# Sanoojan/REFace

Hardware: AMD Instinct MI355X
Metric: 512x512 50-step DDIM images/sec (higher is better)
Workload: dtype bf16; 1 GPU; BASELINE configs[1]: 512x512, 50 DDIM steps, CFG scale 3.5, batch 8 per GPU, bf16 UNet + fp32 VAE decode (bf16x3 MFMA operands), seeded random-init REFace weights; id=c1:512x512:S50:B8:bf16, batch_per_gpu=8, global_batch=8, ddim_steps=50, latent=64, parallelism=dp1 (pairs sharded, no collective in the step loop)

## Files before the change

### include/reface_hip.h

```cpp
#ifndef REFACE_HIP_H
#define REFACE_HIP_H

#include <stdint.h>

#ifdef __cplusplus
extern "C" {
#endif

enum { RF_F32 = 0, RF_BF16 = 1, RF_FP8_E4M3 = 2 ,
       RF_BF16X3 = 3 ,
       RF_F16 = 4  };

enum { RF_ACT_NONE = 0, RF_ACT_GEGLU = 1, RF_ACT_SILU = 2, RF_ACT_QUICK_GELU = 3, RF_ACT_GELU = 4,
       RF_ACT_RELU = 5, RF_ACT_SIGMOID = 6, RF_ACT_PRELU = 7, RF_ACT_ADD_RELU = 8 };

const char* rf_last_error(void);
int rf_version(void);

typedef struct rf_conv_gemm_desc {
    int32_t dtype;
    int32_t out_dtype;
    int32_t M, N, K;
    const void* src0;
    const void* src1;
// ... 73 lines not shown
    void* x1; int32_t ldx1;
} rf_ffn_desc;
int rf_ffn_block(const rf_ffn_desc* d, void* stream);

typedef struct rf_attn_in_desc {
    const void* x; int32_t ldx;
    const void* wpi; int64_t w_sample_stride;
    const float* rowvec; int32_t ldv, rows_per_sample;
    void* tok; int32_t ldt;
    const void* wqkv; const float* bqkv;
    void* qkv; int32_t ldq;
    int32_t M, C;
    float ln_eps;
    int32_t dtype;
} rf_attn_in_desc;
int rf_attn_in(const rf_attn_in_desc* d, void* stream);

int rf_quantize_fp8_rows(const float* w, int N, int K, int ldq, void* q, float* scale, void* stream);

int rf_groupnorm_stats(int dtype, const void* x, int B, int HW, int C, int ldx, int nchunks, double* partial, void* stream);
int rf_groupnorm_finalize(const double* partial_in, int B, int nchunks, double* partial_out, void* stream);
int rf_groupnorm_apply(int dtype, const void* x, int B, int HW, int C, int ldx, int nchunks, const double* partial,
                       const float* gamma, const float* beta, float eps, int silu, int out_dtype, void* out, int ldo, void* stream);
int rf_groupnorm_fold_linear(const float* W, int N, int C, int B, int HW, int nchunks, const double* partial, const float* gamma, const float* beta,
                             const float* bias, float eps, int out_dtype, void* w_out, float* rowvec_out, void* stream);

int rf_gn_silu_conv3x3_small(int dtype, const void* x, int B, int H, int W, int C, int ldx, int nchunks, const double* partial, const float* gamma,
                             const float* beta, float eps, int silu, const void* w, const float* bias, int No, int out_dtype, void* out, int ldo,
                             float* workspace, long long workspace_bytes, void* stream);

typedef struct rf_stem_desc {
    const void* x; int32_t ldx;
    int32_t B, H, W, C;
    const void* w; const float* bias;
    void* out; int32_t ldo;
    long long dup_off;
    double* gn_part0;
    int32_t gn_cpg0, gn_coff0, gn_slot0, gn_nchunks0;
    double* gn_part1;
    int32_t gn_cpg1, gn_coff1, gn_slot1, gn_nchunks1;
    double* gn_part2;
    int32_t gn_cpg2, gn_coff2, gn_slot2, gn_nchunks2;
    int32_t dtype;
} rf_stem_desc;
int rf_conv3x3_stem(const rf_stem_desc* d, void* stream);

// ... 151 lines not shown
```

### reface_amd/_lib.py

```python
import ctypes as C
import os

HERE = os.path.dirname(os.path.abspath(__file__))
LIB_PATH = os.environ.get("REFACE_HIP_LIB") or os.path.join(HERE, "lib", "libreface_hip.so")

RF_F32, RF_BF16, RF_FP8_E4M3, RF_BF16X3, RF_F16 = 0, 1, 2, 3, 4
ACT_NONE, ACT_GEGLU, ACT_SILU, ACT_QUICK_GELU, ACT_GELU, ACT_RELU, ACT_SIGMOID, ACT_PRELU, ACT_ADD_RELU = 0, 1, 2, 3, 4, 5, 6, 7, 8


class ConvGemmDesc(C.Structure):
    _fields_ = [
        ("dtype", C.c_int32), ("out_dtype", C.c_int32),
        ("M", C.c_int32), ("N", C.c_int32), ("K", C.c_int32),
        ("src0", C.c_void_p), ("src1", C.c_void_p),
        ("C0", C.c_int32), ("C1", C.c_int32), ("ld0", C.c_int32), ("ld1", C.c_int32),
        ("Hin", C.c_int32), ("Win", C.c_int32), ("Hout", C.c_int32), ("Wout", C.c_int32),
        ("KH", C.c_int32), ("KW", C.c_int32), ("stride", C.c_int32), ("pad_t", C.c_int32), ("pad_l", C.c_int32),
        ("ups", C.c_int32),
        ("W", C.c_void_p), ("ldw", C.c_int32), ("bias", C.c_void_p), ("rowvec", C.c_void_p),
        ("rows_per_sample", C.c_int32), ("ldv", C.c_int32),
        ("residual", C.c_void_p), ("ldr", C.c_int32), ("act", C.c_int32),
        ("out", C.c_void_p), ("ldo", C.c_int32), ("alpha", C.c_float),
        ("batch", C.c_int32),
        ("sA", C.c_int64), ("sW", C.c_int64), ("sO", C.c_int64), ("sR", C.c_int64),
# ... 58 lines not shown
        ("gn_part0", C.c_void_p), ("gn_cpg0", C.c_int32), ("gn_coff0", C.c_int32), ("gn_slot0", C.c_int32), ("gn_nchunks0", C.c_int32),
        ("gn_part1", C.c_void_p), ("gn_cpg1", C.c_int32), ("gn_coff1", C.c_int32), ("gn_slot1", C.c_int32), ("gn_nchunks1", C.c_int32),
        ("gn_part2", C.c_void_p), ("gn_cpg2", C.c_int32), ("gn_coff2", C.c_int32), ("gn_slot2", C.c_int32), ("gn_nchunks2", C.c_int32),
        ("dtype", C.c_int32),
    ]


_SIGS = {
    "rf_last_error": (C.c_char_p, []),
    "rf_version": (C.c_int, []),
    "rf_conv_gemm": (C.c_int, [C.POINTER(ConvGemmDesc), C.c_void_p]),
    "rf_conv_gemm_plan": (C.c_int, [C.POINTER(ConvGemmDesc), C.POINTER(C.c_int32), C.POINTER(C.c_int32), C.POINTER(C.c_int32)]),
    "rf_conv_gemm_plan2": (C.c_int, [C.POINTER(ConvGemmDesc), C.POINTER(C.c_int32)]),
    "rf_conv_gemm_plan3": (C.c_int, [C.POINTER(ConvGemmDesc), C.POINTER(C.c_int32)]),
    "rf_ffn_geglu": (C.c_int, [C.c_void_p, C.c_int, C.c_void_p, C.c_void_p, C.c_void_p, C.c_void_p, C.c_void_p, C.c_int, C.c_void_p, C.c_int,
                               C.c_int, C.c_int, C.c_float, C.c_void_p]),
    "rf_ffn_block": (C.c_int, [C.POINTER(FfnDesc), C.c_void_p]),
    "rf_attn_in": (C.c_int, [C.POINTER(AttnInDesc), C.c_void_p]),
    "rf_quantize_fp8_rows": (C.c_int, [C.c_void_p, C.c_int, C.c_int, C.c_int, C.c_void_p, C.c_void_p, C.c_void_p]),
    "rf_groupnorm_stats": (C.c_int, [C.c_int, C.c_void_p, C.c_int, C.c_int, C.c_int, C.c_int, C.c_int, C.c_void_p, C.c_void_p]),
    "rf_groupnorm_finalize": (C.c_int, [C.c_void_p, C.c_int, C.c_int, C.c_void_p, C.c_void_p]),
    "rf_groupnorm_apply": (C.c_int, [C.c_int, C.c_void_p, C.c_int, C.c_int, C.c_int, C.c_int, C.c_int, C.c_void_p, C.c_void_p,
                                     C.c_void_p, C.c_float, C.c_int, C.c_int, C.c_void_p, C.c_int, C.c_void_p]),
    "rf_groupnorm_fold_linear": (C.c_int, [C.c_void_p, C.c_int, C.c_int, C.c_int, C.c_int, C.c_int, C.c_void_p, C.c_void_p, C.c_void_p, C.c_void_p,
                                           C.c_float, C.c_int, C.c_void_p, C.c_void_p, C.c_void_p]),
    "rf_gn_silu_conv3x3_small": (C.c_int, [C.c_int, C.c_void_p, C.c_int, C.c_int, C.c_int, C.c_int, C.c_int, C.c_int, C.c_void_p, C.c_void_p, C.c_void_p, C.c_float, C.c_int,
                                           C.c_void_p, C.c_void_p, C.c_int, C.c_int, C.c_void_p, C.c_int, C.c_void_p, C.c_longlong, C.c_void_p]),
    "rf_conv3x3_stem": (C.c_int, [C.POINTER(StemDesc), C.c_void_p]),
    "rf_quantize_fp8_act": (C.c_int, [C.c_void_p, C.c_int64, C.c_int, C.c_int, C.c_void_p, C.c_int, C.c_void_p, C.c_int, C.c_void_p]),
    "rf_groupnorm_apply_fp8": (C.c_int, [C.c_void_p, C.c_int, C.c_int, C.c_int, C.c_int, C.c_int, C.c_void_p, C.c_void_p, C.c_void_p, C.c_float,
                                         C.c_int, C.c_void_p, C.c_int, C.c_void_p, C.c_int, C.c_void_p]),
    "rf_layernorm_fp8": (C.c_int, [C.c_void_p, C.c_int, C.c_int, C.c_int, C.c_void_p, C.c_void_p, C.c_float, C.c_void_p, C.c_int, C.c_void_p, C.c_int,
                                   C.c_void_p]),
    "rf_layernorm": (C.c_int, [C.c_int, C.c_void_p, C.c_int, C.c_int, C.c_int, C.c_void_p, C.c_void_p, C.c_float, C.c_int,
                               C.c_void_p, C.c_int, C.c_void_p]),
    "rf_attention": (C.c_int, [C.c_int, C.c_void_p, C.c_void_p, C.c_void_p, C.c_void_p, C.c_int, C.c_int, C.c_int, C.c_int, C.c_int,
                               C.c_int, C.c_int, C.c_int, C.c_int, C.c_int64, C.c_int64, C.c_int64, C.c_int64, C.c_float, C.c_void_p]),
    "rf_attention_plan": (C.c_int, [C.c_int, C.c_int, C.c_int, C.c_int, C.c_int, C.c_int, C.POINTER(C.c_int32)]),
    "rf_softmax_rows": (C.c_int, [C.c_void_p, C.c_int, C.c_int, C.c_int, C.c_void_p]),
    "rf_ddim_pack_input": (C.c_int, [C.c_void_p, C.c_void_p, C.c_void_p, C.c_int, C.c_int, C.c_int, C.c_int, C.c_void_p, C.c_int, C.c_void_p]),
    "rf_ddim_update": (C.c_int, [C.c_void_p, C.c_int, C.c_int, C.c_float, C.c_void_p, C.c_void_p, C.c_void_p, C.c_int, C.c_int,
                                 C.c_void_p, C.c_void_p]),
    "rf_dpm_update": (C.c_int, [C.c_void_p, C.c_int, C.c_int, C.c_float, C.c_void_p, C.c_void_p, C.c_void_p, C.c_int, C.c_int,
                                C.c_void_p, C.c_void_p]),
    "rf_nchw_to_nhwc": (C.c_int, [C.c_void_p, C.c_int, C.c_int, C.c_int, C.c_int, C.c_void_p, C.c_int, C.c_void_p]),
    "rf_nhwc_to_nchw": (C.c_int, [C.c_int, C.c_void_p, C.c_int, C.c_int, C.c_int, C.c_int, C.c_void_p, C.c_void_p]),
# ... 114 lines not shown
```

### reface_amd/csrc/norm.hip

```cpp
#include <stdarg.h>

#include "common.h"

namespace rf {

static thread_local char g_err[512] = "";
void set_error(const char* fmt, ...) {
    va_list ap;
    va_start(ap, fmt);
    vsnprintf(g_err, sizeof(g_err), fmt, ap);
    va_end(ap);
}

constexpr int GN_SLOTS = 4;
constexpr int GN_THREADS = 256;

template <typename T> struct gn_acc { typedef float type; };
template <> struct gn_acc<float> { typedef double type; };

template <typename T, int NS>
__global__ __launch_bounds__(GN_THREADS) void gn_stats_kernel(const T* __restrict__ x, int HW, int C, int ldx, int nchunks,
                                                              double* __restrict__ partial) {
    typedef typename gn_acc<T>::type acc_t;
    constexpr int VEC = elem<T>::VEC;
    const int nvec = C / VEC;
    const int TV = nvec < GN_THREADS ? nvec : GN_THREADS;
    const int PL = GN_THREADS / TV;
    const int tv = threadIdx.x % TV, pl = threadIdx.x / TV;
    const int b = blockIdx.y, chunk = blockIdx.x;
    const int ppc = (HW + nchunks - 1) / nchunks;
    const int p0 = chunk * ppc, p1 = min(HW, p0 + ppc);
    const int cpg = C / 32;

    constexpr bool SHIFTED = sizeof(T) == 2;
    acc_t s[NS][VEC], ss[NS][VEC];
    float k0[NS][VEC];
    int npix = 0;
#pragma unroll
    for (int q = 0; q < NS; ++q)
#pragma unroll
        for (int e = 0; e < VEC; ++e) { s[q][e] = ss[q][e] = 0; k0[q][e] = 0.f; }

    if (pl < PL) {
        int p = p0 + pl;
        if (SHIFTED && p < p1) {
            const T* row = x + ((long long)b * HW + p) * ldx;
#pragma unroll
            for (int q = 0; q < NS; ++q) {
                const int v = tv + q * TV;
                if (v < nvec) unpack16<T>(*(const u32x4_t*)(row + v * VEC), k0[q]);
            }
            npix = 1;
            p += PL;
        }
        for (; p < p1; p += PL) {
            const T* row = x + ((long long)b * HW + p) * ldx;
#pragma unroll
            for (int q = 0; q < NS; ++q) {
                const int v = tv + q * TV;
                if (v < nvec) {
                    float f[VEC];
                    unpack16<T>(*(const u32x4_t*)(row + v * VEC), f);
#pragma unroll
                    for (int e = 0; e < VEC; ++e) {
                        if constexpr (SHIFTED) {
                            const float d = f[e] - k0[q][e];
                            s[q][e] += d;
                            ss[q][e] += d * d;
                        } else {
                            s[q][e] += f[e];
                            ss[q][e] += (acc_t)f[e] * f[e];
                        }
                    }
                }
            }
            ++npix;
        }
    }
    extern __shared__ __attribute__((aligned(16))) char gn_smem[];
// ... 22 lines not shown
    __shared__ double red[GN_THREADS][2];
    {
        const int g = threadIdx.x & 31, part = threadIdx.x >> 5;
        double a = 0.0, qq = 0.0;
        const int n = PL * cpg;
        for (int e = part; e < n; e += GN_THREADS / 32) {
            const int pp = e / cpg, cc = e - pp * cpg;
            a += chs[pp * C + g * cpg + cc];
            qq += chq[pp * C + g * cpg + cc];
        }
        red[threadIdx.x][0] = a;
        red[threadIdx.x][1] = qq;
    }
    __syncthreads();
    if (threadIdx.x < 32) {
        double sa = 0.0, sq = 0.0;
        for (int k = 0; k < GN_THREADS / 32; ++k) { sa += red[threadIdx.x + 32 * k][0]; sq += red[threadIdx.x + 32 * k][1]; }
        double* o = partial + (((long long)b * nchunks + chunk) * 32 + threadIdx.x) * 2;
        o[0] = sa;
        o[1] = sq;
    }
}

template <typename T, typename TO, int NS>
__global__ __launch_bounds__(GN_THREADS) void gn_apply_kernel(const T* __restrict__ x, int HW, int C, int ldx, int nchunks,
                                                              const double* __restrict__ partial, const float* __restrict__ gamma,
                                                              const float* __restrict__ beta, float eps, int do_silu,
                                                              TO* __restrict__ out, int ldo, int achunks, int split,
                                                              fp8_t* __restrict__ sc_out = nullptr, int lds_sc = 0) {
    constexpr int VEC = elem<T>::VEC;
    const int nvec = C / VEC;
    const int TV = nvec < GN_THREADS ? nvec : GN_THREADS;
    const int PL = GN_THREADS / TV;
    const int tv = threadIdx.x % TV, pl = threadIdx.x / TV;
    const int b = blockIdx.y;
    const int cpg = C / 32;

    __shared__ float mean_s[32], rstd_s[32];
    __shared__ double red[GN_THREADS][2];
    const int ppc = (HW + achunks - 1) / achunks;
    const int p0 = blockIdx.x * ppc, p1 = min(HW, p0 + ppc);
    float gm[NS][VEC], bt[NS][VEC];
    u32x4_t raw0[NS];
#pragma unroll
    for (int q = 0; q < NS; ++q) {
        const int v = tv + q * TV;
#pragma unroll
        for (int e = 0; e < VEC; ++e) { gm[q][e] = 0.f; bt[q][e] = 0.f; }
        raw0[q] = u32x4_t{0u, 0u, 0u, 0u};
        if (v < nvec) {
#pragma unroll
            for (int e = 0; e < VEC; e += 4) {
                const f32x4_t g4 = *(const f32x4_t*)(gamma + v * VEC + e), b4 = *(const f32x4_t*)(beta + v * VEC + e);
                gm[q][e] = g4[0]; gm[q][e + 1] = g4[1]; gm[q][e + 2] = g4[2]; gm[q][e + 3] = g4[3];
                bt[q][e] = b4[0]; bt[q][e + 1] = b4[1]; bt[q][e + 2] = b4[2]; bt[q][e + 3] = b4[3];
            }
            if (pl < PL && p0 + pl < p1) raw0[q] = *(const u32x4_t*)(x + ((long long)b * HW + p0 + pl) * ldx + v * VEC);
        }
    }
    {
        const int g = threadIdx.x & 31, part = threadIdx.x >> 5;
        double a = 0.0, q = 0.0;
#pragma unroll 4
        for (int c = part; c < nchunks; c += GN_THREADS / 32) {
            const double* pp = partial + (((long long)b * nchunks + c) * 32 + g) * 2;
            a += pp[0];
            q += pp[1];
        }
        red[threadIdx.x][0] = a;
        red[threadIdx.x][1] = q;
        __syncthreads();
        if (threadIdx.x < 32) {
            double sa = 0.0, sq = 0.0;
            for (int k = 0; k < GN_THREADS / 32; ++k) { sa += red[threadIdx.x + 32 * k][0]; sq += red[threadIdx.x + 32 * k][1]; }
            const double n = (double)HW * cpg;
            const double mean = sa / n;
            double var = sq / n - mean * mean;
            if (var < 0.0) var = 0.0;
            mean_s[threadIdx.x] = (float)mean;
            rstd_s[threadIdx.x] = (float)(1.0 / sqrt(var + (double)eps));
        }
        __syncthreads();
    }
    float sc[NS][VEC], sh[NS][VEC];
#pragma unroll
    for (int q = 0; q < NS; ++q) {
        const int v = tv + q * TV;
#pragma unroll
        for (int e = 0; e < VEC; ++e) {
            sc[q][e] = sh[q][e] = 0.f;
            if (v < nvec) {
                const int c = v * VEC + e, g = c / cpg;
                const float a = rstd_s[g] * gm[q][e];
                sc[q][e] = a;
                sh[q][e] = bt[q][e] - mean_s[g] * a;
            }
        }
    }
    if (pl >= PL) return;
    u32x4_t cur[NS];
#pragma unroll
    for (int q = 0; q < NS; ++q) cur[q] = raw0[q];
    for (int p = p0 + pl; p < p1; p += PL) {
        const T* nrow = x + ((long long)b * HW + p + PL) * ldx;
        TO* orow = out + ((long long)b * HW + p) * ldo;
        u32x4_t nxt[NS];
#pragma unroll
        for (int q = 0; q < NS; ++q) {
            const int v = tv + q * TV;
            nxt[q] = u32x4_t{0u, 0u, 0u, 0u};
            if (v < nvec && p + PL < p1) nxt[q] = *(const u32x4_t*)(nrow + v * VEC);
        }
#pragma unroll
        for (int q = 0; q < NS; ++q) {
            const int v = tv + q * TV;
            if (v < nvec) {
                float f[VEC];
                unpack16<T>(cur[q], f);
#pragma unroll
                for (int e = 0; e < VEC; ++e) {
                    float y = f[e] * sc[q][e] + sh[q][e];
                    f[e] = do_silu ? silu_exact(y) : y;
                }
                if constexpr (sizeof(TO) == 1) {
                    quant_block8(f, orow + v * VEC, sc_out + ((long long)b * HW + p) * lds_sc + (v >> 2), (v & 3) == 0);
                } else if constexpr (sizeof(TO) == sizeof(T)) {
                    *(u32x4_t*)(orow + v * VEC) = pack16<TO>(f);
                } else if constexpr (sizeof(TO) == 4) {
                    *(u32x4_t*)(orow + v * VEC) = pack16<float>(f);
                    *(u32x4_t*)(orow + v * VEC + 4) = pack16<float>(f + 4);
                } else {
                    u32x2_t h, l;
                    split4_bf16(f, h, l);
                    *(u32x2_t*)(orow + v * VEC) = h;
                    if (split) *(u32x2_t*)(orow + C + v * VEC) = l;
                }
            }
        }
#pragma unroll
        for (int q = 0; q < NS; ++q) cur[q] = nxt[q];
    }
// ... 102 lines not shown
    __syncthreads();
    float s = 0.f;
    for (int c = threadIdx.x * 4; c < cols; c += 1024) {
        const f32x4_t v = *(const f32x4_t*)(r + c);
        s += expf(v[0] - m) + expf(v[1] - m) + expf(v[2] - m) + expf(v[3] - m);
    }
    s = wave_sum(s);
    if ((threadIdx.x & 63) == 0) red[threadIdx.x >> 6] = s;
    __syncthreads();
    const float inv = 1.0f / (red[0] + red[1] + red[2] + red[3]);
    for (int c = threadIdx.x * 4; c < cols; c += 1024) {
        f32x4_t v = *(const f32x4_t*)(r + c);
#pragma unroll
        for (int e = 0; e < 4; ++e) v[e] = expf(v[e] - m) * inv;
        *(f32x4_t*)(r + c) = v;
    }
}

}

using namespace rf;

extern "C" const char* rf_last_error(void) { return rf::g_err; }
extern "C" int rf_version(void) { return 111; }

static int gn_check(const char* name, int dtype, int C, int ldx, int nchunks) {
    const int vec = dtype == RF_F32 ? 4 : 8;
    RF_CHECK(dtype == RF_F32 || dtype == RF_BF16 || dtype == RF_F16, "%s: bad dtype %d", name, dtype);
    RF_CHECK(C % 32 == 0 && C % vec == 0 && ldx % vec == 0, "%s: C=%d ld=%d must be multiples of 32 and %d", name, C, ldx, vec);
    RF_CHECK(C / vec <= GN_SLOTS * GN_THREADS, "%s: C=%d too large", name, C);
    RF_CHECK(nchunks >= 1, "%s: nchunks=%d", name, nchunks);
    return 0;
}

extern "C" int rf_groupnorm_stats(int dtype, const void* x, int B, int HW, int C, int ldx, int nchunks, double* partial, void* stream) {
    if (gn_check("rf_groupnorm_stats", dtype, C, ldx, nchunks)) return 1;
    RF_CHECK(x && partial && B > 0 && HW > 0, "rf_groupnorm_stats: bad arguments");
    dim3 grid(nchunks, B);
    const int vec = dtype == RF_F32 ? 4 : 8;
    const int nvec = C / vec, TV = nvec < GN_THREADS ? nvec : GN_THREADS, PL = GN_THREADS / TV;
    const size_t smem = (size_t)2 * PL * C * sizeof(double);
    RF_CHECK(smem <= 64 * 1024, "rf_groupnorm_stats: C=%d needs %zu B of LDS", C, smem);
    const int ns = (nvec + GN_THREADS - 1) / GN_THREADS;
#define GN_STATS_(T, NS_) hipLaunchKernelGGL((gn_stats_kernel<T, NS_>), grid, dim3(GN_THREADS), smem, (hipStream_t)stream, (const T*)x, HW, C, ldx, nchunks, partial)
#define GN_STATS(T) { if (ns <= 1) GN_STATS_(T, 1); else if (ns <= 2) GN_STATS_(T, 2); else GN_STATS_(T, GN_SLOTS); }
    if (dtype == RF_F32) GN_STATS(float)
    else if (dtype == RF_F16) GN_STATS(f16_t)
// ... 42 lines not shown
    RF_CHECK(!split || (dtype == RF_F32 && ldo >= 2 * C), "rf_groupnorm_apply: split-bf16 output needs fp32 input and ldo >= 2C");
    RF_CHECK(ldo % 8 == 0, "rf_groupnorm_apply: ldo=%d must be a multiple of 8", ldo);
    int achunks = (1024 + B - 1) / B;
    const int maxc = (HW + 1) / 2;
    if (achunks > maxc) achunks = maxc;
    if (achunks < 1) achunks = 1;
    dim3 grid(achunks, B);
    hipStream_t st = (hipStream_t)stream;
    const int ns = (C / (dtype == RF_F32 ? 4 : 8) + GN_THREADS - 1) / GN_THREADS;
#define GN_APPLY_(T, TO, NS_) hipLaunchKernelGGL((gn_apply_kernel<T, TO, NS_>), grid, dim3(GN_THREADS), 0, st, (const T*)x, HW, C, ldx, nchunks, partial, gamma, beta, eps, silu, (TO*)out, ldo, achunks, split)
#define GN_APPLY(T, TO) { if (ns <= 1) GN_APPLY_(T, TO, 1); else if (ns <= 2) GN_APPLY_(T, TO, 2); else GN_APPLY_(T, TO, GN_SLOTS); }
    if (dtype == RF_F32 && out_dtype == RF_F32) GN_APPLY(float, float)
    else if (dtype == RF_F16 && out_dtype == RF_F32) GN_APPLY(f16_t, float)
    else if (dtype == RF_F16) GN_APPLY(f16_t, f16_t)
    else if (dtype == RF_F32) GN_APPLY(float, bf16_t)
    else if (out_dtype == RF_F32) GN_APPLY(bf16_t, float)
    else GN_APPLY(bf16_t, bf16_t)
#undef GN_APPLY
#undef GN_APPLY_
    RF_LAUNCH_CHECK("rf_groupnorm_apply");
    return 0;
}

constexpr int GN_FOLD_RPW = 2;
typedef float f32x2_t __attribute__((ext_vector_type(2)));
template <typename TO, int NIT>
__global__ __launch_bounds__(GN_THREADS) void gn_fold_linear_kernel(const float* __restrict__ W, int N, int C, int HW, int nchunks,
                                                                    const double* __restrict__ partial, const float* __restrict__ gamma,
                                                                    const float* __restrict__ beta, const float* __restrict__ bias, float eps,
                                                                    TO* __restrict__ wout, float* __restrict__ rvout) {
    const int b = blockIdx.y, cpg = C / 32;
    const int lane = threadIdx.x & 63, wave = threadIdx.x >> 6;
    const int n0 = (blockIdx.x * (GN_THREADS / 64) + wave) * GN_FOLD_RPW;
    f32x4_t w8[GN_FOLD_RPW][NIT][2], g8[NIT][2], b8[NIT][2];
#pragma unroll
    for (int it = 0; it < NIT; ++it) {
        const int k = 8 * lane + 512 * it;
#pragma unroll
        for (int h = 0; h < 2; ++h) {
            g8[it][h] = b8[it][h] = f32x4_t{0.f, 0.f, 0.f, 0.f};
            if (k < C) { g8[it][h] = *(const f32x4_t*)(gamma + k + 4 * h); b8[it][h] = *(const f32x4_t*)(beta + k + 4 * h); }
#pragma unroll
            for (int r = 0; r < GN_FOLD_RPW; ++r) {
                w8[r][it][h] = f32x4_t{0.f, 0.f, 0.f, 0.f};
                if (k < C && n0 + r < N) w8[r][it][h] = *(const f32x4_t*)(W + (long long)(n0 + r) * C + k + 4 * h);
            }
// ... 183 lines not shown
```

### reface_amd/ops.py

```python
import ctypes as C
import threading

import torch

from . import _lib
from ._lib import (ACT_ADD_RELU, ACT_GEGLU, ACT_GELU, ACT_NONE, ACT_PRELU, ACT_QUICK_GELU, ACT_RELU, ACT_SIGMOID, ACT_SILU, RF_BF16, RF_BF16X3, RF_F16, RF_F32,
                   RF_FP8_E4M3, AttnInDesc, ConvGemmDesc, FfnDesc, StemDesc)

LOG2E = 1.4426950408889634
LN2 = 0.6931471805599453


def code(dt):
    if dt == torch.float32:
        return RF_F32
    if dt == torch.bfloat16:
        return RF_BF16
    if dt == torch.float16:
        return RF_F16
    raise TypeError(f"unsupported dtype {dt}")


H16 = (torch.bfloat16, torch.float16)

# ... 515 lines not shown
    B, H, W_, Cc = x.shape
    n = gn_chunks(B, H * W_)
    _require_gpu(x, partial)
    assert partial.dtype == torch.float64 and partial.numel() >= B * n * 64
    return Launch(lib.rf_groupnorm_stats, (code(x.dtype), _p(x), B, H * W_, Cc, x.stride(2), n, _p(partial)), (x, partial), name + ".stats"), n


def groupnorm(x, gamma, beta, out, partial, *, eps, silu, split=False, name="groupnorm"):
    lib = _lib.load()
    B, H, W_, Cc = x.shape
    HW = H * W_
    n = gn_chunks(B, HW)
    assert partial.dtype == torch.float64 and partial.numel() >= B * n * 64
    a = Launch(lib.rf_groupnorm_stats, (code(x.dtype), _p(x), B, HW, Cc, x.stride(2), n, _p(partial)), (x, partial), name + ".stats")
    if isinstance(out, Fp8Act):
        return [a, groupnorm_apply(x, gamma, beta, out, partial, n, eps=eps, silu=silu, name=name)]
    _require_gpu(x, gamma, beta, out, partial)
    b = Launch(lib.rf_groupnorm_apply, (code(x.dtype), _p(x), B, HW, Cc, x.stride(2), n, _p(partial), _p(gamma), _p(beta),
                                        float(eps), int(bool(silu)), _gn_out_code(x, out, split), _p(out), out.stride(2)),
               (x, partial, gamma, beta, out), name + ".apply")
    return [a, b]


def gemm_plan(launch):
    pl = gemm_plan3(launch, ".plan")
    return pl["stat_rows"], pl["stat_cols"], pl["splitk"]


PLAN2_KEYS = ("stat_rows", "stat_cols", "splitk", "bm", "bn", "wave_cols", "direct", "frag", "gemm_kernels")


def gemm_plan2(launch):
    pl = gemm_plan3(launch, ".plan2")
    return {k: pl[k] for k in PLAN2_KEYS}


REDUCE_KINDS = ("none", "stripe8", "stripe32", "frag")


def gemm_plan3(launch, what=".plan3"):
    lib = _lib.load()
    info = (C.c_int32 * 24)()
    _lib.check(lib.rf_conv_gemm_plan3(C.byref(launch.keep[0]), info), launch.name + what)
    v = [int(x) for x in info]
    pl = dict(zip(PLAN2_KEYS[:8], v[:8]))
    pl["gemm_kernels"] = 2 if pl["frag"] & 2 else 1
# ... 733 lines not shown
```

### reface_amd/vae.py

```python
import os

import torch
import torch.nn as nn

from . import ops
from .gnfuse import ProducerTracker
from .modules import ParamTree, flat_state, weights_version
from .params import VAEConfig, vae_param_specs
from .unet import _Pool

F32 = torch.float32


class DiagonalGaussianDistribution(object):

    def __init__(self, parameters, deterministic=False):
        self.parameters = parameters
        self.deterministic = deterministic

    @property
    def mean(self):
        return torch.chunk(self.parameters, 2, dim=1)[0]

    @property
# ... 4 lines not shown
        B, C2, H, W = self.parameters.shape
        out = torch.empty((B, C2 // 2, H, W), dtype=F32, device=self.parameters.device)
        ops.gaussian_sample(self.parameters.contiguous(), eps, out, scale=scale)()
        return out

    def sample(self, noise=None, scale=1.0):
        if self.deterministic:
            return self._draw(None, scale)
        if noise is None:
            noise = torch.randn(self.mean.shape)
        return self._draw(noise.to(device=self.parameters.device, dtype=F32).contiguous(), scale)

    def mode(self):
        return self._draw(None, 1.0)


class _VAEEngine:
    def __init__(self, sd, cfg: VAEConfig, B, H, W, dtype, device, which):
        self.x3 = dtype == "bf16x3"
        if self.x3:
            dtype = F32
        self.cfg, self.B, self.dt, self.dev = cfg, B, dtype, device
        self.n_x3 = 0
        self.pool = _Pool(device)
        self.tracker = ProducerTracker()
        self.pool.on_put = self.tracker.forget
        self.gn_fuse = os.environ.get("REFACE_GN_FUSE", "1") == "1"
        self.gn_fused = 0
        self.sd = {k: v.detach().to(device=device, dtype=F32) for k, v in sd.items()}
        self.gn_partial = torch.empty(B * ops.GN_MAX_CHUNKS * 64, dtype=torch.float64, device=device)
        self.launches = []
        self.ws = ops.new_workspace(device)
        with ops.workspace_scope(self.ws):
            (self._build_decoder if which == "dec" else self._build_encoder)(H, W)
        self.sd = None

    def w(self, key):
        return self.sd[key].to(self.dt).contiguous()

    def f32(self, key):
        return self.sd[key].contiguous()

    def _x3_ok(self, cin, ksize=3):
        return self.x3 and ops.x3_eligible(ksize * ksize * cin, cin)

    def _split(self, x):
        B, H, W, c = x.shape
        s = self.pool.get((B, H, W, 2 * c), torch.bfloat16)
        self.launches.append(ops.split_bf16(x, s, name="split_bf16"))
        return s

    def _gn(self, x, key, silu=True, split=False):
        out = self.pool.get(tuple(x.shape[:3]) + (2 * x.shape[3],), torch.bfloat16) if split else self.pool.get(tuple(x.shape), self.dt)
# ... 13 lines not shown
        return out

    def _conv3(self, key, x, cout, *, cin_pad=None, stride=1, pad=(1, 1), ups=0, residual=None, out=None):
        B, H, W, _ = x.shape
        Ho, Wo = (2 * H, 2 * W) if ups else ((H // 2, W // 2) if stride == 2 else (H, W))
        y = out if out is not None else self.pool.get((B, Ho, Wo, cout), self.dt)
        x3 = self.x3 and x.dtype == torch.bfloat16
        wp = ops.pack_conv_weight(self.sd[key + ".weight"], F32 if x3 else self.dt, cin_pad=cin_pad)
        if x3:
            wp = ops.pack_x3(wp)
            self.n_x3 += 1
        self._conv(x, wp, y, self.f32(key + ".bias"), stride=stride, pad=pad, ups=ups, residual=residual, x3=x3, name=key)
        return y

    def _conv(self, x, wp, y, bias, residual=None, **kw):
        B, n = x.shape[0], 1
        while (x.numel() // n) * x.element_size() >= 0x7fff0000 and B % (2 * n) == 0:
            n *= 2
        step = B // n
        for i in range(n):
            sl = slice(i * step, (i + 1) * step)
            self.launches.append(self.tracker.record(y[sl], ops.conv2d(x[sl], wp, y[sl], bias, residual=None if residual is None else residual[sl], **kw)))

    def _res(self, p, x, cin, cout):
        B, H, W, _ = x.shape
        t1 = self._gn(x, f"{p}.norm1", split=self._x3_ok(cin))
        h1 = self._conv3(f"{p}.conv1", t1, cout)
        self.pool.put(t1)
        t2 = self._gn(h1, f"{p}.norm2", split=self._x3_ok(cout))
        self.pool.put(h1)
        if cin != cout:
            sc = self.pool.get((B, H, W, cout), self.dt)
            if self._x3_ok(cin, 1):
                xs = self._split(x)
                self._conv(xs, ops.pack_x3(self.sd[f"{p}.nin_shortcut.weight"].reshape(cout, cin)), sc,
                           self.f32(f"{p}.nin_shortcut.bias"), ksize=1, pad=(0, 0), x3=True, name=f"{p}.nin_shortcut")
                self.pool.put(xs)
                self.n_x3 += 1
            else:
                self._conv(x, self.w(f"{p}.nin_shortcut.weight").reshape(cout, cin), sc,
                           self.f32(f"{p}.nin_shortcut.bias"), ksize=1, pad=(0, 0), name=f"{p}.nin_shortcut")
        else:
            sc = x
        y = self._conv3(f"{p}.conv2", t2, cout, residual=sc)
        self.pool.put(t2)
        if cin != cout:
            self.pool.put(sc)
        return y

    def _attn(self, p, x, c):
        B, H, W, _ = x.shape
        N = H * W
        M = B * N
        g = self._gn(x, f"{p}.norm", silu=False)
        g2 = g.view(M, c)
        wq, wk, wv = (self.sd[f"{p}.{n}.weight"].reshape(c, c) for n in ("q", "k", "v"))
        qk = self.pool.get((M, 2 * c), self.dt)
        self.launches.append(ops.linear(g2, torch.cat([wq, wk], 0).to(self.dt).contiguous(), qk,
                                        torch.cat([self.sd[f"{p}.q.bias"], self.sd[f"{p}.k.bias"]]).contiguous(), name=f"{p}.qk"))
        vt = self.pool.get((B, c, N), self.dt)
        self.launches.append(ops.conv_gemm(wv.to(self.dt).contiguous(), g2, vt, M=c, N=N, K=c, C0=c, ld0=c, Hin=1, Win=c, Hout=1, Wout=c,
                                           ldo=N, batch=B, sA=0, sW=N * c, sO=c * N, name=f"{p}.vT"))
        scores = self.pool.get((B, N, N), F32)
        self.launches.append(ops.conv_gemm(qk, qk[:, c:], scores, M=N, N=N, K=c, C0=c, ld0=2 * c, Hin=1, Win=N, Hout=1, Wout=N,
                                           ldo=N, alpha=float(int(c) ** (-0.5)), batch=B, sA=N * 2 * c, sW=N * 2 * c, sO=N * N, ldw=2 * c,
                                           name=f"{p}.scores"))
        self.launches.append(ops.softmax_rows(scores.view(B * N, N), name=f"{p}.softmax"))
        if self.dt != F32:
            probs = self.pool.get((B, N, N), self.dt)
            self.launches.append(ops.cast(scores, probs))
# ... 20 lines not shown

    def _build_decoder(self, h, w):
        cfg, B, dev = self.cfg, self.B, self.dev
        ZP = 8
        self.z_in = torch.empty((B, cfg.embed_dim, h, w), dtype=F32, device=dev)
        z_cl = torch.zeros((B, h, w, ZP), dtype=self.dt, device=dev)
        self.launches.append(ops.nchw_to_nhwc(self.z_in, z_cl))
        zq = torch.zeros((B, h, w, ZP), dtype=self.dt, device=dev)
        wpq = torch.zeros((cfg.z_channels, ZP), dtype=F32, device=dev)
        wpq[:, :cfg.embed_dim] = self.sd["post_quant_conv.weight"].reshape(cfg.z_channels, cfg.embed_dim)
        self.pq_alpha_launch_index = len(self.launches)
        self._pq = (z_cl, wpq.to(self.dt).contiguous(), zq)
        self.launches.append(None)
        nres = len(cfg.ch_mult)
        block_in = cfg.ch * cfg.ch_mult[nres - 1]
        hcur = self._conv3("decoder.conv_in", zq, block_in, cin_pad=ZP)
        hcur = self._mid("decoder.mid", hcur, block_in)
        for lvl in reversed(range(nres)):
            block_out = cfg.ch * cfg.ch_mult[lvl]
            for b in range(cfg.num_res_blocks + 1):
                nh = self._res(f"decoder.up.{lvl}.block.{b}", hcur, block_in, block_out)
                self.pool.put(hcur)
                hcur, block_in = nh, block_out
            if lvl != 0:
                hs = self._split(hcur) if self._x3_ok(block_in) else hcur
                nh = self._conv3(f"decoder.up.{lvl}.upsample.conv", hs, block_in, ups=1)
                if hs is not hcur:
                    self.pool.put(hs)
                self.pool.put(hcur)
                hcur = nh
        g = self._gn(hcur, "decoder.norm_out", split=self._x3_ok(block_in))
        self.pool.put(hcur)
        H, W = g.shape[1], g.shape[2]
        out4 = torch.empty((B, H, W, 4), dtype=F32, device=dev)
        self._conv3("decoder.conv_out", g, cfg.out_ch, out=out4[..., :cfg.out_ch])
        self.out = torch.empty((B, cfg.out_ch, H, W), dtype=F32, device=dev)
        self.launches.append(ops.nhwc_to_nchw(out4, self.out, C_=cfg.out_ch))
        self.set_scale(1.0)

    def set_scale(self, inv_scale):
        z_cl, wpq, zq = self._pq
        B, h, w, ZP = z_cl.shape
        self.launches[self.pq_alpha_launch_index] = ops.conv_gemm(
            z_cl, wpq, zq, M=B * h * w, N=self.cfg.z_channels, K=ZP, C0=ZP, ld0=ZP, Hin=1, Win=B * h * w, Hout=1, Wout=B * h * w,
            bias=self._pq_bias(), ldo=ZP, alpha=float(inv_scale), name="post_quant_conv")

    def _pq_bias(self):
# ... 105 lines not shown
```

Before: 10.32 images/s.

## Fold VAE upsample conv into four phase 2x2 convs with phase-aware groupnorm

Replaces the nearest-upsample plus 3x3 conv in the VAE decoder with four sub-pixel phase convolutions using folded 2x2 weights. The result stays in a phase-major layout, and new groupnorm stats/apply kernels read that layout directly. The apply kernel also writes the raw fp32 or split-bf16 activations in normal layout, so the following resblock can use them for its residual or shortcut. This is meant to cut the FLOPs and memory traffic of convolving an upsampled tensor, and to remove a separate split pass. The cost is extra kernel complexity and strided gathers.

```diff
diff --git a/include/reface_hip.h b/include/reface_hip.h
--- a/include/reface_hip.h
+++ b/include/reface_hip.h
@@ -119,6 +119,10 @@
 int rf_groupnorm_finalize(const double* partial_in, int B, int nchunks, double* partial_out, void* stream);
 int rf_groupnorm_apply(int dtype, const void* x, int B, int HW, int C, int ldx, int nchunks, const double* partial,
                        const float* gamma, const float* beta, float eps, int silu, int out_dtype, void* out, int ldo, void* stream);
+int rf_groupnorm_stats_ph(const float* x, int B, int Hs, int Ws, int C, int ldx, int nchunks, double* partial, void* stream);
+int rf_groupnorm_apply_ph(const float* x, int B, int Hs, int Ws, int C, int ldx, int nchunks, const double* partial, const float* gamma,
+                          const float* beta, float eps, int silu, void* out, int ldo, float* raw_out, int ldr, void* raw_split_out, int lds,
+                          void* stream);
 int rf_groupnorm_fold_linear(const float* W, int N, int C, int B, int HW, int nchunks, const double* partial, const float* gamma, const float* beta,
                              const float* bias, float eps, int out_dtype, void* w_out, float* rowvec_out, void* stream);
 
diff --git a/reface_amd/_lib.py b/reface_amd/_lib.py
--- a/reface_amd/_lib.py
+++ b/reface_amd/_lib.py
@@ -104,6 +104,9 @@
     "rf_groupnorm_finalize": (C.c_int, [C.c_void_p, C.c_int, C.c_int, C.c_void_p, C.c_void_p]),
     "rf_groupnorm_apply": (C.c_int, [C.c_int, C.c_void_p, C.c_int, C.c_int, C.c_int, C.c_int, C.c_int, C.c_void_p, C.c_void_p,
                                      C.c_void_p, C.c_float, C.c_int, C.c_int, C.c_void_p, C.c_int, C.c_void_p]),
+    "rf_groupnorm_stats_ph": (C.c_int, [C.c_void_p, C.c_int, C.c_int, C.c_int, C.c_int, C.c_int, C.c_int, C.c_void_p, C.c_void_p]),
+    "rf_groupnorm_apply_ph": (C.c_int, [C.c_void_p, C.c_int, C.c_int, C.c_int, C.c_int, C.c_int, C.c_int, C.c_void_p, C.c_void_p, C.c_void_p,
+                                        C.c_float, C.c_int, C.c_void_p, C.c_int, C.c_void_p, C.c_int, C.c_void_p, C.c_int, C.c_void_p]),
     "rf_groupnorm_fold_linear": (C.c_int, [C.c_void_p, C.c_int, C.c_int, C.c_int, C.c_int, C.c_int, C.c_void_p, C.c_void_p, C.c_void_p, C.c_void_p,
                                            C.c_float, C.c_int, C.c_void_p, C.c_void_p, C.c_void_p]),
     "rf_gn_silu_conv3x3_small": (C.c_int, [C.c_int, C.c_void_p, C.c_int, C.c_int, C.c_int, C.c_int, C.c_int, C.c_int, C.c_void_p, C.c_void_p, C.c_void_p, C.c_float, C.c_int,
diff --git a/reface_amd/csrc/norm.hip b/reface_amd/csrc/norm.hip
--- a/reface_amd/csrc/norm.hip
+++ b/reface_amd/csrc/norm.hip
@@ -15,12 +15,20 @@
 constexpr int GN_SLOTS = 4;
 constexpr int GN_THREADS = 256;
 
+struct gn_ph {
+    int w = 0, hw = 0;
+    float* raw_out = nullptr;
+    int ldr = 0;
+    bf16_t* raw_split = nullptr;
+    int lds = 0;
+};
+
 template <typename T> struct gn_acc { typedef float type; };
 template <> struct gn_acc<float> { typedef double type; };
 
-template <typename T, int NS>
+template <typename T, int NS, bool PH = false>
 __global__ __launch_bounds__(GN_THREADS) void gn_stats_kernel(const T* __restrict__ x, int HW, int C, int ldx, int nchunks,
-                                                              double* __restrict__ partial) {
+                                                              double* __restrict__ partial, const gn_ph ph = gn_ph()) {
     typedef typename gn_acc<T>::type acc_t;
     constexpr int VEC = elem<T>::VEC;
     const int nvec = C / VEC;
@@ -32,7 +40,15 @@
     const int p0 = chunk * ppc, p1 = min(HW, p0 + ppc);
     const int cpg = C / 32;
 
+    auto row_of = [&](int p) -> const T* {
+        if constexpr (PH) {
+            const int f = p / ph.hw;
+            return x + ((long long)(f * (int)gridDim.y + b) * ph.hw + (p - f * ph.hw)) * ldx;
+        }
+        return x + ((long long)b * HW + p) * ldx;
+    };
     constexpr bool SHIFTED = sizeof(T) == 2;
+    static_assert(!PH || !SHIFTED, "phase-major sources are fp32");
     acc_t s[NS][VEC], ss[NS][VEC];
     float k0[NS][VEC];
     int npix = 0;
@@ -44,7 +60,7 @@
     if (pl < PL) {
         int p = p0 + pl;
         if (SHIFTED && p < p1) {
-            const T* row = x + ((long long)b * HW + p) * ldx;
+            const T* row = row_of(p);
 #pragma unroll
             for (int q = 0; q < NS; ++q) {
                 const int v = tv + q * TV;
@@ -53,8 +69,37 @@
             npix = 1;
             p += PL;
         }
+        if constexpr (PH) {
+            constexpr int U = 4;
+            for (; p + (U - 1) * PL < p1; p += U * PL) {
+                u32x4_t r[U][NS];
+#pragma unroll
+                for (int u = 0; u < U; ++u) {
+                    const T* row = row_of(p + u * PL);
+#pragma unroll
+                    for (int q = 0; q < NS; ++q) {
+                        const int v = tv + q * TV;
+                        r[u][q] = u32x4_t{0u, 0u, 0u, 0u};
+                        if (v < nvec) r[u][q] = *(const u32x4_t*)(row + v * VEC);
+                    }
+                }
+#pragma unroll
+                for (int u = 0; u < U; ++u)
+#pragma unroll
+                    for (int q = 0; q < NS; ++q) {
+                        float f[VEC];
+                        unpack16<T>(r[u][q], f);
+#pragma unroll
+                        for (int e = 0; e < VEC; ++e) {
+                            s[q][e] += f[e];
+                            ss[q][e] += (acc_t)f[e] * f[e];
+                        }
+                    }
+                npix += U;
+            }
+        }
         for (; p < p1; p += PL) {
-            const T* row = x + ((long long)b * HW + p) * ldx;
+            const T* row = row_of(p);
 #pragma unroll
             for (int q = 0; q < NS; ++q) {
                 const int v = tv + q * TV;
@@ -123,12 +168,12 @@
     }
 }
 
-template <typename T, typename TO, int NS>
+template <typename T, typename TO, int NS, bool PH = false>
 __global__ __launch_bounds__(GN_THREADS) void gn_apply_kernel(const T* __restrict__ x, int HW, int C, int ldx, int nchunks,
                                                               const double* __restrict__ partial, const float* __restrict__ gamma,
                                                               const float* __restrict__ beta, float eps, int do_silu,
                                                               TO* __restrict__ out, int ldo, int achunks, int split,
-                                                              fp8_t* __restrict__ sc_out = nullptr, int lds_sc = 0) {
+                                                              fp8_t* __restrict__ sc_out = nullptr, int lds_sc = 0, const gn_ph ph = gn_ph()) {
     constexpr int VEC = elem<T>::VEC;
     const int nvec = C / VEC;
     const int TV = nvec < GN_THREADS ? nvec : GN_THREADS;
@@ -136,6 +181,13 @@
     const int tv = threadIdx.x % TV, pl = threadIdx.x / TV;
     const int b = blockIdx.y;
     const int cpg = C / 32;
+    auto row_of = [&](int p) -> const T* {
+        if constexpr (PH) {
+            const int W2 = 2 * ph.w, Y = p / W2, X = p - Y * W2;
+            return x + ((long long)((2 * (Y & 1) + (X & 1)) * (int)gridDim.y + b) * ph.hw + (Y >> 1) * ph.w + (X >> 1)) * ldx;
+        }
+        return x + ((long long)b * HW + p) * ldx;
+    };
 
     __shared__ float mean_s[32], rstd_s[32];
     __shared__ double red[GN_THREADS][2];
@@ -156,7 +208,7 @@
                 gm[q][e] = g4[0]; gm[q][e + 1] = g4[1]; gm[q][e + 2] = g4[2]; gm[q][e + 3] = g4[3];
                 bt[q][e] = b4[0]; bt[q][e + 1] = b4[1]; bt[q][e + 2] = b4[2]; bt[q][e + 3] = b4[3];
             }
-            if (pl < PL && p0 + pl < p1) raw0[q] = *(const u32x4_t*)(x + ((long long)b * HW + p0 + pl) * ldx + v * VEC);
+            if (pl < PL && p0 + pl < p1) raw0[q] = *(const u32x4_t*)(row_of(p0 + pl) + v * VEC);
         }
     }
     {
@@ -203,7 +255,7 @@
 #pragma unroll
     for (int q = 0; q < NS; ++q) cur[q] = raw0[q];
     for (int p = p0 + pl; p < p1; p += PL) {
-        const T* nrow = x + ((long long)b * HW + p + PL) * ldx;
+        const T* nrow = row_of(p + PL);
         TO* orow = out + ((long long)b * HW + p) * ldo;
         u32x4_t nxt[NS];
 #pragma unroll
@@ -218,6 +270,16 @@
             if (v < nvec) {
                 float f[VEC];
                 unpack16<T>(cur[q], f);
+                if constexpr (PH) {
+                    if (ph.raw_out) *(u32x4_t*)(ph.raw_out + ((long long)b * HW + p) * ph.ldr + v * VEC) = cur[q];
+                    if (ph.raw_split) {
+                        bf16_t* const srow = ph.raw_split + ((long long)b * HW + p) * ph.lds;
+                        u32x2_t h, l;
+                        split4_bf16(f, h, l);
+                        *(u32x2_t*)(srow + v * VEC) = h;
+                        *(u32x2_t*)(srow + C + v * VEC) = l;
+                    }
+                }
 #pragma unroll
                 for (int e = 0; e < VEC; ++e) {
                     float y = f[e] * sc[q][e] + sh[q][e];
@@ -366,7 +428,7 @@
 using namespace rf;
 
 extern "C" const char* rf_last_error(void) { return rf::g_err; }
-extern "C" int rf_version(void) { return 111; }
+extern "C" int rf_version(void) { return 112; }
 
 static int gn_check(const char* name, int dtype, int C, int ldx, int nchunks) {
     const int vec = dtype == RF_F32 ? 4 : 8;
@@ -455,6 +517,64 @@
     return 0;
 }
 
+static int gn_ph_check(const char* name, const void* x, int B, int Hs, int Ws, int C, int ldx, int nchunks) {
+    if (gn_check(name, RF_F32, C, ldx, nchunks)) return 1;
+    RF_CHECK(x && B > 0 && Hs > 0 && Ws > 0 && ldx >= C, "%s: bad arguments B=%d Hs=%d Ws=%d C=%d ldx=%d", name, B, Hs, Ws, C, ldx);
+    RF_CHECK((long long)Hs * Ws <= (1 << 28) && 4ll * B * Hs * Ws < (1ll << 31), "%s: %d x %d x %d phase pixels exceed the 31-bit pixel index", name, B, Hs, Ws);
+    RF_CHECK(((uintptr_t)x & 15) == 0, "%s: the source must be 16-byte aligned", name);
+    return 0;
+}
+
+extern "C" int rf_groupnorm_stats_ph(const float* x, int B, int Hs, int Ws, int C, int ldx, int nchunks, double* partial, void* stream) {
+    if (gn_ph_check("rf_groupnorm_stats_ph", x, B, Hs, Ws, C, ldx, nchunks)) return 1;
+    RF_CHECK(partial, "rf_groupnorm_stats_ph: bad arguments");
+    gn_ph ph;
+    ph.w = Ws;
+    ph.hw = Hs * Ws;
+    const int HW = 4 * ph.hw;
+    dim3 grid(nchunks, B);
+    const int nvec = C / 4, TV = nvec < GN_THREADS ? nvec : GN_THREADS, PL = GN_THREADS / TV;
+    const size_t smem = (size_t)2 * PL * C * sizeof(double);
+    RF_CHECK(smem <= 64 * 1024, "rf_groupnorm_stats_ph: C=%d needs %zu B of LDS", C, smem);
+    const int ns = (nvec + GN_THREADS - 1) / GN_THREADS;
+#define GN_STATS_PH_(NS_) hipLaunchKernelGGL((gn_stats_kernel<float, NS_, true>), grid, dim3(GN_THREADS), smem, (hipStream_t)stream, x, HW, C, ldx, nchunks, partial, ph)
+    if (ns <= 1) GN_STATS_PH_(1); else if (ns <= 2) GN_STATS_PH_(2); else GN_STATS_PH_(GN_SLOTS);
+#undef GN_STATS_PH_
+    RF_LAUNCH_CHECK("rf_groupnorm_stats_ph");
+    return 0;
+}
+
+extern "C" int rf_groupnorm_apply_ph(const float* x, int B, int Hs, int Ws, int C, int ldx, int nchunks, const double* partial, const float* gamma,
+                                     const float* beta, float eps, int silu, void* out, int ldo, float* raw_out, int ldr, void* raw_split_out, int lds,
+                                     void* stream) {
+    if (gn_ph_check("rf_groupnorm_apply_ph", x, B, Hs, Ws, C, ldx, nchunks)) return 1;
+    RF_CHECK(partial && gamma && beta && out, "rf_groupnorm_apply_ph: bad arguments");
+    RF_CHECK((((uintptr_t)gamma | (uintptr_t)beta) & 15) == 0, "rf_groupnorm_apply_ph: gamma / beta must be 16-byte aligned");
+    RF_CHECK(ldo >= 2 * C && ldo % 8 == 0 && ((uintptr_t)out & 7) == 0, "rf_groupnorm_apply_ph: the split-bf16 output needs ldo=%d >= 2C, a multiple of 8, and 8-byte alignment", ldo);
+    RF_CHECK(!raw_out || (ldr >= C && ldr % 4 == 0 && ((uintptr_t)raw_out & 15) == 0), "rf_groupnorm_apply_ph: raw_out needs ldr=%d >= C, a multiple of 4, and 16-byte alignment", ldr);
+    RF_CHECK(!raw_split_out || (lds >= 2 * C && lds % 4 == 0 && ((uintptr_t)raw_split_out & 7) == 0),
+             "rf_groupnorm_apply_ph: raw_split_out needs lds=%d >= 2C, a multiple of 4, and 8-byte alignment", lds);
+    gn_ph ph;
+    ph.w = Ws;
+    ph.hw = Hs * Ws;
+    ph.raw_out = raw_out;
+    ph.ldr = ldr;
+    ph.raw_split = (bf16_t*)raw_split_out;
+    ph.lds = lds;
+    const int HW = 4 * ph.hw;
+    int achunks = (1024 + B - 1) / B;
+    const int maxc = (HW + 1) / 2;
+    if (achunks > maxc) achunks = maxc;
+    if (achunks < 1) achunks = 1;
+    dim3 grid(achunks, B);
+    const int ns = (C / 4 + GN_THREADS - 1) / GN_THREADS;
+#define GN_APPLY_PH_(NS_) hipLaunchKernelGGL((gn_apply_kernel<float, bf16_t, NS_, true>), grid, dim3(GN_THREADS), 0, (hipStream_t)stream, x, HW, C, ldx, nchunks, partial, gamma, beta, eps, silu, (bf16_t*)out, ldo, achunks, 1, (fp8_t*)nullptr, 0, ph)
+    if (ns <= 1) GN_APPLY_PH_(1); else if (ns <= 2) GN_APPLY_PH_(2); else GN_APPLY_PH_(GN_SLOTS);
+#undef GN_APPLY_PH_
+    RF_LAUNCH_CHECK("rf_groupnorm_apply_ph");
+    return 0;
+}
+
 constexpr int GN_FOLD_RPW = 2;
 typedef float f32x2_t __attribute__((ext_vector_type(2)));
 template <typename TO, int NIT>
diff --git a/reface_amd/ops.py b/reface_amd/ops.py
--- a/reface_amd/ops.py
+++ b/reface_amd/ops.py
@@ -561,6 +561,56 @@
     return [a, b]
 
 
+def phase_index_map(B, H, W):
+    b = torch.arange(B).view(B, 1, 1)
+    Y = torch.arange(2 * H).view(1, 2 * H, 1)
+    X = torch.arange(2 * W).view(1, 1, 2 * W)
+    return ((2 * (Y & 1) + (X & 1)) * B + b) * (H * W) + (Y >> 1) * W + (X >> 1)
+
+
+def pack_ups_phases_x3(w):
+    f = fold_ups_weight(w)
+    return [pack_x3(f[p].reshape(f.shape[1], 4 * f.shape[4])) for p in range(4)]
+
+
+def ups_phase_pad(p):
+    return (1 - (p >> 1), 1 - (p & 1))
+
+
+GN_PH_MAX_CHUNKS = GN_FUSED_MAX_CHUNKS
+
+
+def gn_chunks_ph(B, HW):
+    return max(1, min(GN_PH_MAX_CHUNKS, HW // 32, 1024 // B))
+
+
+def groupnorm_stats_ph(P, partial, name="groupnorm"):
+    lib = _lib.load()
+    _, B, H, W_, Cc = P.shape
+    n = gn_chunks_ph(B, 4 * H * W_)
+    _require_gpu(P, partial)
+    assert P.dtype == torch.float32 and P.is_contiguous() and partial.dtype == torch.float64 and partial.numel() >= B * n * 64
+    return Launch(lib.rf_groupnorm_stats_ph, (_p(P), B, H, W_, Cc, Cc, n, _p(partial)), (P, partial), name + ".stats"), n
+
+
+def groupnorm_apply_ph(P, gamma, beta, out, partial, nchunks, *, eps, silu, raw_out=None, raw_split_out=None, name="groupnorm"):
+    lib = _lib.load()
+    _, B, H, W_, Cc = P.shape
+    _require_gpu(P, gamma, beta, out, partial, raw_out, raw_split_out)
+    assert P.dtype == torch.float32 and P.is_contiguous()
+    for t, dt, c in ((out, torch.bfloat16, 2 * Cc), (raw_out, torch.float32, Cc), (raw_split_out, torch.bfloat16, 2 * Cc)):
+        assert t is None or (t.dtype == dt and tuple(t.shape) == (B, 2 * H, 2 * W_, c) and t.is_contiguous()), (None if t is None else tuple(t.shape), dt, c)
+    return Launch(lib.rf_groupnorm_apply_ph, (_p(P), B, H, W_, Cc, Cc, nchunks, _p(partial), _p(gamma), _p(beta), float(eps), int(bool(silu)),
+                                              _p(out), out.stride(2), _p(raw_out), 0 if raw_out is None else raw_out.stride(2),
+                                              _p(raw_split_out), 0 if raw_split_out is None else raw_split_out.stride(2)),
+                  (P, partial, gamma, beta, out, raw_out, raw_split_out), name + ".apply")
+
+
+def groupnorm_ph(P, gamma, beta, out, partial, *, eps, silu, raw_out=None, raw_split_out=None, name="groupnorm"):
+    a, n = groupnorm_stats_ph(P, partial, name)
+    return [a, groupnorm_apply_ph(P, gamma, beta, out, partial, n, eps=eps, silu=silu, raw_out=raw_out, raw_split_out=raw_split_out, name=name)]
+
+
 def gemm_plan(launch):
     pl = gemm_plan3(launch, ".plan")
     return pl["stat_rows"], pl["stat_cols"], pl["splitk"]
diff --git a/reface_amd/vae.py b/reface_amd/vae.py
--- a/reface_amd/vae.py
+++ b/reface_amd/vae.py
@@ -50,13 +50,15 @@
             dtype = F32
         self.cfg, self.B, self.dt, self.dev = cfg, B, dtype, device
         self.n_x3 = 0
+        self.ups_fold = os.environ.get("REFACE_VAE_UPS_FOLD", "1") == "1"
+        self.n_ups_folded = 0
         self.pool = _Pool(device)
         self.tracker = ProducerTracker()
         self.pool.on_put = self.tracker.forget
         self.gn_fuse = os.environ.get("REFACE_GN_FUSE", "1") == "1"
         self.gn_fused = 0
         self.sd = {k: v.detach().to(device=device, dtype=F32) for k, v in sd.items()}
-        self.gn_partial = torch.empty(B * ops.GN_MAX_CHUNKS * 64, dtype=torch.float64, device=device)
+        self.gn_partial = torch.empty(B * max(ops.GN_MAX_CHUNKS, ops.GN_PH_MAX_CHUNKS) * 64, dtype=torch.float64, device=device)
         self.launches = []
         self.ws = ops.new_workspace(device)
         with ops.workspace_scope(self.ws):
@@ -116,9 +118,34 @@
             sl = slice(i * step, (i + 1) * step)
             self.launches.append(self.tracker.record(y[sl], ops.conv2d(x[sl], wp, y[sl], bias, residual=None if residual is None else residual[sl], **kw)))
 
+    def _ups_phases(self, key, x, c):
+        B, H, W, _ = x.shape
+        xs = self._split(x)
+        P = self.pool.get((4, B, H, W, c), F32)
+        wps = ops.pack_ups_phases_x3(self.sd[key + ".weight"])
+        for ph in range(4):
+            self._conv(xs, wps[ph], P[ph], self.f32(key + ".bias"), ksize=2, stride=1, pad=ops.ups_phase_pad(ph), x3=True, name=f"{key}.ph{ph}")
+        self.pool.put(xs)
+        self.n_x3 += 1
+        self.n_ups_folded += 1
+        return P
+
     def _res(self, p, x, cin, cout):
-        B, H, W, _ = x.shape
-        t1 = self._gn(x, f"{p}.norm1", split=self._x3_ok(cin))
+        xs = raw = None
+        if x.dim() == 5:
+            _, B, H, W, _ = x.shape
+            H, W = 2 * H, 2 * W
+            t1 = self.pool.get((B, H, W, 2 * cin), torch.bfloat16)
+            if cin == cout:
+                raw = self.pool.get((B, H, W, cin), F32)
+            else:
+                xs = self.pool.get((B, H, W, 2 * cin), torch.bfloat16)
+            self.launches += ops.groupnorm_ph(x, self.f32(f"{p}.norm1.weight"), self.f32(f"{p}.norm1.bias"), t1, self.gn_partial, eps=1e-6,
+                                              silu=True, raw_out=raw, raw_split_out=xs, name=f"{p}.norm1")
+            x = raw
+        else:
+            B, H, W, _ = x.shape
+            t1 = self._gn(x, f"{p}.norm1", split=self._x3_ok(cin))
         h1 = self._conv3(f"{p}.conv1", t1, cout)
         self.pool.put(t1)
         t2 = self._gn(h1, f"{p}.norm2", split=self._x3_ok(cout))
@@ -126,7 +153,8 @@
         if cin != cout:
             sc = self.pool.get((B, H, W, cout), self.dt)
             if self._x3_ok(cin, 1):
-                xs = self._split(x)
+                if xs is None:
+                    xs = self._split(x)
                 self._conv(xs, ops.pack_x3(self.sd[f"{p}.nin_shortcut.weight"].reshape(cout, cin)), sc,
                            self.f32(f"{p}.nin_shortcut.bias"), ksize=1, pad=(0, 0), x3=True, name=f"{p}.nin_shortcut")
                 self.pool.put(xs)
@@ -140,6 +168,8 @@
         self.pool.put(t2)
         if cin != cout:
             self.pool.put(sc)
+        if raw is not None:
+            self.pool.put(raw)
         return y
 
     def _attn(self, p, x, c):
@@ -206,7 +236,11 @@
                 nh = self._res(f"decoder.up.{lvl}.block.{b}", hcur, block_in, block_out)
                 self.pool.put(hcur)
                 hcur, block_in = nh, block_out
-            if lvl != 0:
+            if lvl != 0 and self.x3 and self.ups_fold and self._x3_ok(block_in):
+                nh = self._ups_phases(f"decoder.up.{lvl}.upsample.conv", hcur, block_in)
+                self.pool.put(hcur)
+                hcur = nh
+            elif lvl != 0:
                 hs = self._split(hcur) if self._x3_ok(block_in) else hcur
                 nh = self._conv3(f"decoder.up.{lvl}.upsample.conv", hs, block_in, ups=1)
                 if hs is not hcur:
```

Result: no change. 10.41 images/s (median of 6 runs) (+0.9%).
